# eth-cscs/conflux

Measured on NVIDIA H100. Metric: LU GFLOP/s (FP64, (2/3)N^3), higher is better.
Workload: dtype f64

## Files before the change

conflux_b200/csrc/gemm.cu:

```cuda
#include <cstdlib>

#include "common.cuh"
#include "kernels.h"

namespace cflx {

namespace {
constexpr int BK = 16, STAGES = 4;

template <int WM, int WN>
struct Cfg {
    static constexpr int BM = 64 * WM, BN = 32 * WN;
    static constexpr int LDA = BM + 4, LDB = BN + 4;
    static constexpr int NCONS = WM * WN, NTHREADS = (NCONS + 1) * 32;
    static constexpr size_t SMEM = (size_t)STAGES * BK * (LDA + LDB) * sizeof(double) + 2 * STAGES * sizeof(uint64_t);
};

__device__ __forceinline__ double2 ld_c2(const double* p) {
    double2 v;
    asm("ld.global.v2.f64 {%0, %1}, [%2];" : "=d"(v.x), "=d"(v.y) : "l"(p));
    return v;
}

template <int WM, int WN, int MINB>
__global__ void __launch_bounds__(Cfg<WM, WN>::NTHREADS, MINB) gemm_tn_kernel(GemmArgs g) {
    using C = Cfg<WM, WN>;
    constexpr int BM = C::BM, BN = C::BN, LDA = C::LDA, LDB = C::LDB, NCONS = C::NCONS;
    extern __shared__ __align__(128) unsigned char smem_raw[];
    double* sA = reinterpret_cast<double*>(smem_raw);
    double* sB = sA + STAGES * BK * LDA;
    uint64_t* full = reinterpret_cast<uint64_t*>(sB + STAGES * BK * LDB);
    uint64_t* empty = full + STAGES;

    const int warp = threadIdx.x >> 5, lane = threadIdx.x & 31;
    const int m0 = blockIdx.y * BM, n0 = blockIdx.x * BN;

    if (threadIdx.x == 0) {
        for (int s = 0; s < STAGES; ++s) {
            mbar_init(&full[s], 1);
            mbar_init(&empty[s], NCONS);
        }
        fence_barrier_init();
    }
    __syncthreads();

    if (warp == NCONS) {
        int wm = g.M - m0;
        wm = wm > BM ? BM : ((wm + 1) & ~1);
        int wn = g.N - n0;
        wn = wn > BN ? BN : ((wn + 1) & ~1);
        const int rr = lane & 15;
        for (int kt = 0; kt * BK < g.K; ++kt) {
            const int s = kt % STAGES, u = kt / STAGES;
            if (u > 0) mbar_wait(&empty[s], (u - 1) & 1);
            const int rows = min(BK, g.K - kt * BK);
            if (lane == 0) mbar_arrive_expect_tx(&full[s], (uint32_t)(rows * (wm + wn) * sizeof(double)));
            __syncwarp();
            if (rr < rows) {
                const int64_t k = (int64_t)kt * BK + rr;
                if (lane < 16)
                    bulk_g2s(sA + (s * BK + rr) * LDA, g.AT + k * g.ldat + m0, (uint32_t)(wm * sizeof(double)), &full[s]);
                else
                    bulk_g2s(sB + (s * BK + rr) * LDB, g.B + k * g.ldb + n0, (uint32_t)(wn * sizeof(double)), &full[s]);
            }
        }
        return;
    }

    const int wm_off = (warp / WN) * 64, wn_off = (warp % WN) * 32;
    const int g4 = lane >> 2, t4 = lane & 3;
    double acc[4][4][4];
#pragma unroll
    for (int i = 0; i < 4; ++i)
#pragma unroll
        for (int j = 0; j < 4; ++j) acc[i][j][0] = acc[i][j][1] = acc[i][j][2] = acc[i][j][3] = 0.0;

    for (int kt = 0; kt * BK < g.K; ++kt) {
        const int s = kt % STAGES, u = kt / STAGES;
        mbar_wait(&full[s], u & 1);
        const double* a_s = sA + s * BK * LDA + wm_off + g4;
        const double* b_s = sB + s * BK * LDB + wn_off + g4;
        const int rows = min(BK, g.K - kt * BK);
#pragma unroll
        for (int kk = 0; kk < BK; kk += 8) {
            if (kk < rows) {
                const bool hi = kk + 4 < rows;
                const double* a_k = a_s + (kk + t4) * LDA;
                const double* b_k = b_s + (kk + t4) * LDB;
                double b[4][2];
#pragma unroll
                for (int j = 0; j < 4; ++j) {
                    b[j][0] = b_k[8 * j];
                    b[j][1] = hi ? b_k[4 * LDB + 8 * j] : 0.0;
                }
#pragma unroll
                for (int i = 0; i < 4; ++i) {
                    const double a[4] = {a_k[16 * i], a_k[16 * i + 8], hi ? a_k[4 * LDA + 16 * i] : 0.0,
                                         hi ? a_k[4 * LDA + 16 * i + 8] : 0.0};
#pragma unroll
                    for (int j = 0; j < 4; ++j) dmma16x8x8(acc[i][j], a, b[j]);
                }
            }
        }
        __syncwarp();
        if (lane == 0) mbar_arrive(&empty[s]);
    }

    const double alpha = g.alpha, beta = g.beta;
    const bool use_c = (beta != 0.0);
    const int row0 = m0 + wm_off + g4, col0 = n0 + wn_off + 2 * t4;
#pragma unroll
    for (int sl = 0; sl < 8; ++sl) {
        const int row = row0 + 8 * sl;
        double2 cv[4];
#pragma unroll
        for (int j = 0; j < 4; ++j) {
            const int col = col0 + 8 * j;
            cv[j] = make_double2(0.0, 0.0);
            if (use_c && row < g.M && col < g.N) cv[j] = ld_c2(g.C + (int64_t)row * g.ldc + col);
        }
#pragma unroll
        for (int j = 0; j < 4; ++j) {
            const int col = col0 + 8 * j;
            if (row < g.M && col < g.N) {
                double2 out;
                out.x = fma(alpha, acc[sl / 2][j][2 * (sl & 1)], beta * cv[j].x);
                out.y = fma(alpha, acc[sl / 2][j][2 * (sl & 1) + 1], beta * cv[j].y);
                *reinterpret_cast<double2*>(g.D + (int64_t)row * g.ldd + col) = out;
            }
        }
    }
}
}

namespace {
template <int WM, int WN, int MINB>
int setup_one() {
    static PerDeviceMax cfg;
    if (cfg.raise(Cfg<WM, WN>::SMEM))
        CFLX_CUDA(cudaFuncSetAttribute(gemm_tn_kernel<WM, WN, MINB>, cudaFuncAttributeMaxDynamicSharedMemorySize,
                                       (int)Cfg<WM, WN>::SMEM));
    return CFLX_OK;
}
template <int WM, int WN, int MINB>
int launch_one(const GemmArgs& g, cudaStream_t stream) {
    using C = Cfg<WM, WN>;
    CFLX_TRY((setup_one<WM, WN, MINB>()));
    dim3 grid((g.N + C::BN - 1) / C::BN, (g.M + C::BM - 1) / C::BM);
    gemm_tn_kernel<WM, WN, MINB><<<grid, C::NTHREADS, C::SMEM, stream>>>(g);
    CFLX_CUDA(cudaGetLastError());
    return CFLX_OK;
}
int tile_variant() {
    static int v = -1;
    if (v < 0) {
        const char* e = getenv("CFLX_GEMM_TILE");
        v = (e && atoi(e) == 64) ? 64 : 128;
    }
    return v;
}
}

int gemm_tn_setup() {
    CFLX_TRY((setup_one<2, 4, 1>()));
    CFLX_TRY((setup_one<1, 4, 2>()));
    return CFLX_OK;
}

int launch_gemm_tn(const GemmArgs& g, cudaStream_t stream) {
    if (g.M <= 0 || g.N <= 0 || g.K <= 0) return CFLX_OK;
    if ((g.K & 3) || (g.N & 1) || (g.ldat & 1) || (g.ldb & 1) || (g.ldc & 1) || (g.ldd & 1)) {
        set_last_error("gemm_tn: unsupported shape M=%d N=%d K=%d ld=(%lld,%lld,%lld,%lld)", g.M, g.N, g.K,
                       (long long)g.ldat, (long long)g.ldb, (long long)g.ldc, (long long)g.ldd);
        return CFLX_ERR_UNSUPPORTED;
    }
    if (tile_variant() == 64) return launch_one<1, 4, 2>(g, stream);
    return launch_one<2, 4, 1>(g, stream);
}

}
```

Measured before the change: 22460.

## Prefetch C tile into freed pipeline stages via bulk copies in 128-row GEMM

For the 128x128 tile variant, the producer warp issues bulk async copies of the C tile into the A/B shared-memory stage buffers as they are released after the last K iterations. Consumer warps then read C from shared memory through per-slab mbarriers instead of issuing global loads in the epilogue. The goal is to hide epilogue C-load latency behind the tail of the mainloop. In exchange it adds barriers and tricky buffer reuse, with a 4*(rr&1) offset to avoid bank conflicts, which raises correctness risk.

```diff
diff --git a/conflux_b200/csrc/gemm.cu b/conflux_b200/csrc/gemm.cu
--- a/conflux_b200/csrc/gemm.cu
+++ b/conflux_b200/csrc/gemm.cu
@@ -13,7 +13,10 @@
     static constexpr int BM = 64 * WM, BN = 32 * WN;
     static constexpr int LDA = BM + 4, LDB = BN + 4;
     static constexpr int NCONS = WM * WN, NTHREADS = (NCONS + 1) * 32;
-    static constexpr size_t SMEM = (size_t)STAGES * BK * (LDA + LDB) * sizeof(double) + 2 * STAGES * sizeof(uint64_t);
+    static constexpr bool STAGE_C = (WM == 2);
+    static constexpr int NBAR = 2 * STAGES + (STAGE_C ? WM * STAGES : 0);
+    static constexpr size_t SMEM = (size_t)STAGES * BK * (LDA + LDB) * sizeof(double) + NBAR * sizeof(uint64_t);
+    static_assert(!STAGE_C || (LDA == LDB && 64 / 16 == STAGES), "one slab per warp row and stage, in both parts");
 };
 
 __device__ __forceinline__ double2 ld_c2(const double* p) {
@@ -31,6 +34,7 @@
     double* sB = sA + STAGES * BK * LDA;
     uint64_t* full = reinterpret_cast<uint64_t*>(sB + STAGES * BK * LDB);
     uint64_t* empty = full + STAGES;
+    uint64_t* cfull = empty + STAGES;
 
     const int warp = threadIdx.x >> 5, lane = threadIdx.x & 31;
     const int m0 = blockIdx.y * BM, n0 = blockIdx.x * BN;
@@ -40,6 +44,8 @@
             mbar_init(&full[s], 1);
             mbar_init(&empty[s], NCONS);
         }
+        if constexpr (C::STAGE_C)
+            for (int b = 0; b < WM * STAGES; ++b) mbar_init(&cfull[b], 1);
         fence_barrier_init();
     }
     __syncthreads();
@@ -50,7 +56,9 @@
         int wn = g.N - n0;
         wn = wn > BN ? BN : ((wn + 1) & ~1);
         const int rr = lane & 15;
-        for (int kt = 0; kt * BK < g.K; ++kt) {
+        const int nkt = (g.K + BK - 1) / BK;
+        const bool use_c = (g.beta != 0.0);
+        for (int kt = 0; kt < nkt; ++kt) {
             const int s = kt % STAGES, u = kt / STAGES;
             if (u > 0) mbar_wait(&empty[s], (u - 1) & 1);
             const int rows = min(BK, g.K - kt * BK);
@@ -64,6 +72,21 @@
                     bulk_g2s(sB + (s * BK + rr) * LDB, g.B + k * g.ldb + n0, (uint32_t)(wn * sizeof(double)), &full[s]);
             }
         }
+        if constexpr (C::STAGE_C) {
+            if (use_c)
+                for (int i = 0; i < STAGES; ++i) {
+                    const int s = (nkt + i) % STAGES, kt = nkt + i - STAGES;
+                    if (kt >= 0) mbar_wait(&empty[s], (kt / STAGES) & 1);
+                    const int wr = lane >> 4, r0 = m0 + 64 * wr + 16 * i;
+                    const int rows = max(0, min(16, g.M - r0));
+                    uint64_t* bar = &cfull[wr * STAGES + i];
+                    if (rr == 0) mbar_arrive_expect_tx(bar, (uint32_t)(rows * wn * sizeof(double)));
+                    __syncwarp();
+                    if (rr < rows)
+                        bulk_g2s(sA + (wr * STAGES + s) * BK * LDA + rr * LDA + 4 * (rr & 1),
+                                 g.C + (int64_t)(r0 + rr) * g.ldc + n0, (uint32_t)(wn * sizeof(double)), bar);
+                }
+        }
         return;
     }
 
@@ -75,7 +98,8 @@
 #pragma unroll
         for (int j = 0; j < 4; ++j) acc[i][j][0] = acc[i][j][1] = acc[i][j][2] = acc[i][j][3] = 0.0;
 
-    for (int kt = 0; kt * BK < g.K; ++kt) {
+    int kt = 0;
+    for (; kt * BK < g.K; ++kt) {
         const int s = kt % STAGES, u = kt / STAGES;
         mbar_wait(&full[s], u & 1);
         const double* a_s = sA + s * BK * LDA + wm_off + g4;
@@ -109,24 +133,49 @@
     const double alpha = g.alpha, beta = g.beta;
     const bool use_c = (beta != 0.0);
     const int row0 = m0 + wm_off + g4, col0 = n0 + wn_off + 2 * t4;
-#pragma unroll
-    for (int sl = 0; sl < 8; ++sl) {
-        const int row = row0 + 8 * sl;
-        double2 cv[4];
-#pragma unroll
-        for (int j = 0; j < 4; ++j) {
-            const int col = col0 + 8 * j;
-            cv[j] = make_double2(0.0, 0.0);
-            if (use_c && row < g.M && col < g.N) cv[j] = ld_c2(g.C + (int64_t)row * g.ldc + col);
-        }
-#pragma unroll
-        for (int j = 0; j < 4; ++j) {
-            const int col = col0 + 8 * j;
-            if (row < g.M && col < g.N) {
-                double2 out;
-                out.x = fma(alpha, acc[sl / 2][j][2 * (sl & 1)], beta * cv[j].x);
-                out.y = fma(alpha, acc[sl / 2][j][2 * (sl & 1) + 1], beta * cv[j].y);
-                *reinterpret_cast<double2*>(g.D + (int64_t)row * g.ldd + col) = out;
+    if constexpr (C::STAGE_C) {
+        const int wr = warp / WN, nkt = kt;
+#pragma unroll
+        for (int i = 0; i < 4; ++i) {
+            const double* cs = sA + (wr * STAGES + (nkt + i) % STAGES) * BK * LDA + 4 * (g4 & 1) + wn_off + 2 * t4;
+            if (use_c) mbar_wait(&cfull[wr * STAGES + i], 0);
+#pragma unroll
+            for (int h = 0; h < 2; ++h) {
+                const int row = row0 + 16 * i + 8 * h;
+#pragma unroll
+                for (int j = 0; j < 4; ++j) {
+                    const int col = col0 + 8 * j;
+                    if (row < g.M && col < g.N) {
+                        double2 cv = make_double2(0.0, 0.0);
+                        if (use_c) cv = *reinterpret_cast<const double2*>(cs + (g4 + 8 * h) * LDA + 8 * j);
+                        double2 out;
+                        out.x = fma(alpha, acc[i][j][2 * h], beta * cv.x);
+                        out.y = fma(alpha, acc[i][j][2 * h + 1], beta * cv.y);
+                        *reinterpret_cast<double2*>(g.D + (int64_t)row * g.ldd + col) = out;
+                    }
+                }
+            }
+        }
+    } else {
+#pragma unroll
+        for (int sl = 0; sl < 8; ++sl) {
+            const int row = row0 + 8 * sl;
+            double2 cv[4];
+#pragma unroll
+            for (int j = 0; j < 4; ++j) {
+                const int col = col0 + 8 * j;
+                cv[j] = make_double2(0.0, 0.0);
+                if (use_c && row < g.M && col < g.N) cv[j] = ld_c2(g.C + (int64_t)row * g.ldc + col);
+            }
+#pragma unroll
+            for (int j = 0; j < 4; ++j) {
+                const int col = col0 + 8 * j;
+                if (row < g.M && col < g.N) {
+                    double2 out;
+                    out.x = fma(alpha, acc[sl / 2][j][2 * (sl & 1)], beta * cv[j].x);
+                    out.y = fma(alpha, acc[sl / 2][j][2 * (sl & 1) + 1], beta * cv[j].y);
+                    *reinterpret_cast<double2*>(g.D + (int64_t)row * g.ldd + col) = out;
+                }
             }
         }
     }
```

After: 23960 (median of 6 runs). +6.7%, better.
